# google-research/big_vision

Measured on NVIDIA H100. Metric: siglip_vit_b16_pairs_per_sec, higher is better.
Workload: dtype bf16

## Files before the change

big_vision_b200/csrc/gemm.cu:

```cuda
#include "common.cuh"
#include "gemm_sched.h"
#include "host_utils.h"

#include <atomic>

#include <stdlib.h>
#include <string.h>

namespace bv {

namespace {

constexpr int BM = 128;
constexpr int BK = 64;
constexpr int A_STAGE_BYTES = BM * BK * 2;
constexpr int NUM_THREADS = 384;
constexpr int SUB_BYTES = 64 * 64 * 2;

enum : int { EF_BIAS = 0, EF_GELU = 1, EF_RESID = 2, EF_DGELU = 3, EF_RESID_ROWMOD = 4, EF_GELU_ACT = 5 };
enum : int { OM_F32 = 0, OM_BF16_ADD = 1, OM_BF16_TMA = 2 };

template <int BN, int OM, int EF>
struct Cfg {
  static constexpr int B_STAGE_BYTES = BN * BK * 2;
  static constexpr int STAGE_BYTES = A_STAGE_BYTES + B_STAGE_BYTES;
  static constexpr bool AUX_TMA = OM == OM_BF16_TMA && (EF == EF_RESID || EF == EF_DGELU);
  static constexpr int OUTS = OM != OM_BF16_TMA ? 0 : (EF == EF_GELU ? 2 : 1);
  static constexpr int BUF_BYTES = OUTS * SUB_BYTES;
  static constexpr int BUFS = AUX_TMA ? BN / 64 : 2;
  static constexpr int STAGING_BYTES = 2 * BUFS * BUF_BYTES;
  static constexpr int SMEM_LIMIT = 232448 - 2048;
  static constexpr int STAGES_FIT = (SMEM_LIMIT - STAGING_BYTES) / STAGE_BYTES;
  static constexpr int STAGES = STAGES_FIT > 8 ? 8 : STAGES_FIT;
  static constexpr int STAGING_OFFSET = STAGES * STAGE_BYTES;
  static constexpr int BAR_OFFSET = STAGING_OFFSET + STAGING_BYTES;
  static constexpr int AUX_BAR = 2 * STAGES;
  static constexpr int SMEM_BYTES = BAR_OFFSET + 256 + 1024;
  static_assert(STAGES >= 3, "shared-memory budget leaves fewer than 3 stages");
  static_assert(8 * (AUX_BAR + (AUX_TMA ? 2 * BUFS : 0)) <= 256, "barriers overflow their 256 bytes");
};

struct GemmDev {
  GemmSched s;
  int M, N;
  int a_mn, b_mn;
  int reduce_out;
  float alpha;
  const float* bias;
  const bf16* aux;
  void* d; void* d2;
  long long ldd, ldd2, ldaux;
  float* colsum;
  int aux_row_mod;
};

template <int BN, int STAGES, int STAGE_BYTES, int TA, int TB, typename F>
__device__ __forceinline__ void mainloop(float (&acc)[BN / 2], uint32_t base, uint32_t bar_base, int cw,
                                         PipeState& ps, int kb0, int kb1, F&& after_first) {
  constexpr uint32_t a_lbo = TA ? 8192u : 16u, b_lbo = TB ? 8192u : 16u;
  constexpr uint32_t a_kstep = TA ? 2048u : 32u, b_kstep = TB ? 2048u : 32u;
  int prev_stage = -1;
  for (int kb = kb0; kb < kb1; ++kb) {
    mbar_wait(bar_base + 8u * ps.stage, ps.phase);
    const uint32_t a_s = base + ps.stage * STAGE_BYTES + cw * 8192;
    const uint32_t b_s = base + ps.stage * STAGE_BYTES + A_STAGE_BYTES;
    const uint64_t adesc = wgmma_desc_sw128(a_s, a_lbo, 1024u), bdesc = wgmma_desc_sw128(b_s, b_lbo, 1024u);
    wgmma_fence_regs(acc);
    wgmma_fence();
#pragma unroll
    for (int k = 0; k < BK / 16; ++k) {
      const uint64_t a = adesc + k * (a_kstep >> 4), b = bdesc + k * (b_kstep >> 4);
      const int accumulate = (kb > kb0 || k > 0) ? 1 : 0;
      if constexpr (BN == 256) wgmma_ss_n256<TA, TB>(acc, a, b, accumulate);
      else wgmma_ss_n128<TA, TB>(acc, a, b, accumulate);
    }
    wgmma_commit();
    wgmma_fence_regs(acc);
    if (kb == kb0) after_first();
    wgmma_wait<1>();
    if (prev_stage >= 0 && (threadIdx.x & 127) == 0) mbar_arrive(bar_base + 8u * (STAGES + prev_stage));
    prev_stage = ps.stage;
    ps.advance(STAGES);
  }
  wgmma_wait<0>();
  wgmma_fence_regs(acc);
  if (prev_stage >= 0 && (threadIdx.x & 127) == 0) mbar_arrive(bar_base + 8u * (STAGES + prev_stage));
}

__device__ __forceinline__ void aux_global(const GemmDev& p, int row, int col, bool pair, float& a0, float& a1) {
  const long long ar = p.aux_row_mod > 0 ? (row % p.aux_row_mod) : row;
  const bf16* ap = p.aux + ar * p.ldaux + col;
  if (pair) {
    const uint32_t q = *reinterpret_cast<const uint32_t*>(ap);
    a0 = bf16_lo(q); a1 = bf16_hi(q);
  } else {
    a0 = __bfloat162float(*ap);
    a1 = 0.f;
  }
}

template <bool OUT_F32, int EF>
__device__ __forceinline__ void epi_math(float alpha, float c0, float c1, float b0, float b1, float a0, float a1,
                                         float& v0, float& v1, float& pre0, float& pre1) {
  v0 = c0 * alpha + b0;
  v1 = c1 * alpha + b1;
  pre0 = pre1 = 0.f;
  if (EF == EF_GELU || EF == EF_GELU_ACT) {
    pre0 = round_bf16(v0); pre1 = round_bf16(v1);
    v0 = gelu_tanh_fast(pre0); v1 = gelu_tanh_fast(pre1);
  } else if (EF == EF_RESID || EF == EF_RESID_ROWMOD) {
    v0 = (OUT_F32 ? v0 : round_bf16(v0)) + a0;
    v1 = (OUT_F32 ? v1 : round_bf16(v1)) + a1;
  } else if (EF == EF_DGELU) {
    v0 *= gelu_tanh_grad_fast(a0);
    v1 *= gelu_tanh_grad_fast(a1);
  }
}


__device__ __forceinline__ void colsum_add(float* colsum, int N, float s0, float s1, int col, int lane) {
  s0 += __shfl_xor_sync(0xffffffffu, s0, 4);
  s0 += __shfl_xor_sync(0xffffffffu, s0, 8);
  s0 += __shfl_xor_sync(0xffffffffu, s0, 16);
  s1 += __shfl_xor_sync(0xffffffffu, s1, 4);
  s1 += __shfl_xor_sync(0xffffffffu, s1, 8);
  s1 += __shfl_xor_sync(0xffffffffu, s1, 16);
  if (lane < 4) {
    if (col < N) atomicAdd(colsum + col, s0);
    if (col + 1 < N) atomicAdd(colsum + col + 1, s1);
  }
}

template <int BN, bool OUT_F32, int EF>
__device__ __forceinline__ void epilogue_regs(const GemmDev& p, const float (&acc)[BN / 2], int m0, int n0,
                                              int cw, int kb0) {
  const int lane = threadIdx.x & 31, warp = (threadIdx.x >> 5) & 3;
  const int row0 = m0 + cw * 64 + warp * 16 + (lane >> 2);
  const int pM = p.M, pN = p.N;
  const float alpha = p.alpha;
  const bool reduce = p.reduce_out != 0;
  const bool first = kb0 == 0;
#pragma unroll
  for (int j = 0; j < BN / 8; ++j) {
    const int col = n0 + 8 * j + 2 * (lane & 3);
    if (col >= pN) continue;
    const bool pair = col + 1 < pN;
    float b0 = 0.f, b1 = 0.f;
    if (p.bias != nullptr && first) {
      b0 = __ldg(p.bias + col);
      if (pair) b1 = __ldg(p.bias + col + 1);
    }
#pragma unroll
    for (int h = 0; h < 2; ++h) {
      const int row = row0 + 8 * h;
      if (row >= pM) continue;
      float v0, v1, pre0, pre1, a0 = 0.f, a1 = 0.f;
      if ((EF == EF_RESID && first) || EF == EF_DGELU) aux_global(p, row, col, pair, a0, a1);
      epi_math<OUT_F32, EF>(alpha, acc[4 * j + 2 * h], acc[4 * j + 2 * h + 1], b0, b1, a0, a1, v0, v1, pre0, pre1);
      if (OUT_F32) {
        float* dp = static_cast<float*>(p.d) + row * p.ldd + col;
        if (reduce) {
          atomicAdd(dp, v0);
          if (pair) atomicAdd(dp + 1, v1);
        } else if (pair) {
          *reinterpret_cast<float2*>(dp) = make_float2(v0, v1);
        } else {
          *dp = v0;
        }
      } else {
        bf16* dp = static_cast<bf16*>(p.d) + row * p.ldd + col;
        const __nv_bfloat162 o = __floats2bfloat162_rn(v0, v1);
        if (pair) atomicAdd(reinterpret_cast<__nv_bfloat162*>(dp), o);
        else atomicAdd(dp, o.x);
      }
    }
  }
}

template <int BN, int EF, int BUF_BYTES>
__device__ __forceinline__ void epilogue_tma(const GemmDev& p, const CUtensorMap* tmD, const CUtensorMap* tmD2,
                                             const float (&acc)[BN / 2], int m0, int n0, int cw, uint32_t staging,
                                             uint32_t& nstore, uint32_t aux_bar, uint32_t aux_parity) {
  constexpr bool AUX_TMA = (EF == EF_RESID || EF == EF_DGELU);
  const int lane = threadIdx.x & 31, warp = (threadIdx.x >> 5) & 3;
  const bool leader = (threadIdx.x & 127) == 0;
  const int rl0 = warp * 16 + (lane >> 2);
  const int row0 = m0 + cw * 64 + rl0;
  const int pM = p.M, pN = p.N, pN8 = p.N & ~7;
  const float alpha = p.alpha;
#pragma unroll
  for (int c = 0; c < BN / 64; ++c) {
    uint32_t buf;
    if constexpr (AUX_TMA) {
      buf = staging + c * BUF_BYTES;
      mbar_wait(aux_bar + 8u * c, aux_parity);
    } else {
      buf = staging + (nstore & 1u) * BUF_BYTES;
      if (leader) tma_store_wait_read<1>();
      named_bar_sync(1 + cw, 128);
    }
    float cs[8][2];
#pragma unroll
    for (int jj = 0; jj < 8; ++jj) {
      const int j = 8 * c + jj;
      const int col = n0 + 8 * j + 2 * (lane & 3);
      cs[jj][0] = cs[jj][1] = 0.f;
      const bool cin = col < pN, pair = col + 1 < pN;
      float b0 = 0.f, b1 = 0.f;
      if (cin && p.bias != nullptr) {
        b0 = __ldg(p.bias + col);
        if (pair) b1 = __ldg(p.bias + col + 1);
      }
#pragma unroll
      for (int h = 0; h < 2; ++h) {
        const int rl = rl0 + 8 * h, row = row0 + 8 * h;
        const uint32_t off = rl * 128 + ((jj ^ (rl & 7)) << 4) + (lane & 3) * 4;
        float v0 = 0.f, v1 = 0.f, pre0 = 0.f, pre1 = 0.f;
        const bool in = cin && row < pM;
        if (in) {
          float a0 = 0.f, a1 = 0.f;
          if constexpr (AUX_TMA) {
            uint32_t q;
            asm volatile("ld.shared.b32 %0, [%1];" : "=r"(q) : "r"(buf + off));
            a0 = bf16_lo(q); a1 = bf16_hi(q);
          } else if constexpr (EF == EF_RESID_ROWMOD) {
            aux_global(p, row, col, pair, a0, a1);
          }
          epi_math<false, EF>(alpha, acc[4 * j + 2 * h], acc[4 * j + 2 * h + 1], b0, b1, a0, a1, v0, v1, pre0, pre1);
        }
        const __nv_bfloat162 o = __floats2bfloat162_rn(v0, v1);
        if (in) {
          cs[jj][0] += __low2float(o);
          cs[jj][1] += pair ? __high2float(o) : 0.f;
        }
        asm volatile("st.shared.b32 [%0], %1;" ::"r"(buf + off), "r"(*reinterpret_cast<const uint32_t*>(&o))
                     : "memory");
        if (EF == EF_GELU) {
          const __nv_bfloat162 q = __floats2bfloat162_rn(pre0, pre1);
          asm volatile("st.shared.b32 [%0], %1;" ::"r"(buf + SUB_BYTES + off),
                       "r"(*reinterpret_cast<const uint32_t*>(&q))
                       : "memory");
        }
      }
    }
    fence_proxy_async();
    named_bar_sync(1 + cw, 128);
    if (leader) {
      if (n0 + 64 * c < pN8 && m0 + cw * 64 < pM) {
        tma_store_2d(tmD, buf, n0 + 64 * c, m0 + cw * 64);
        if (EF == EF_GELU) tma_store_2d(tmD2, buf + SUB_BYTES, n0 + 64 * c, m0 + cw * 64);
      }
      tma_store_commit();
    }
    const int tail0 = pN8 - (n0 + 64 * c);
    if (pN8 < pN && tail0 >= 0 && tail0 < 64) {
      const int t = threadIdx.x & 127, rl = t & 63, out = t >> 6;
      const int row = m0 + cw * 64 + rl;
      if (row < pM && (out == 0 || EF == EF_GELU)) {
        const uint32_t src = buf + out * SUB_BYTES + rl * 128 + (((tail0 >> 3) ^ (rl & 7)) << 4);
        uint16_t* dst = reinterpret_cast<uint16_t*>(out ? p.d2 : p.d) + row * (out ? p.ldd2 : p.ldd) + pN8;
#pragma unroll 1
        for (int e = 0; e < pN - pN8; ++e) {
          uint16_t u;
          asm volatile("ld.shared.u16 %0, [%1];" : "=h"(u) : "r"(src + 2 * e));
          dst[e] = u;
        }
      }
      named_bar_sync(1 + cw, 128);
    }
    if (!AUX_TMA) ++nstore;
    if (p.colsum != nullptr) {
#pragma unroll
      for (int jj = 0; jj < 8; ++jj)
        colsum_add(p.colsum, pN, cs[jj][0], cs[jj][1], n0 + 8 * (8 * c + jj) + 2 * (lane & 3), lane);
    }
  }
}

template <int BN>
__device__ __forceinline__ void issue_aux_loads(const CUtensorMap* tmAux, int M, int N, int m0, int n0, int cw,
                                                uint32_t staging, uint32_t aux_bar) {
  tma_store_wait_read<0>();
#pragma unroll
  for (int c = 0; c < BN / 64; ++c) {
    const uint32_t bar = aux_bar + 8u * c;
    if (n0 + 64 * c < N && m0 + cw * 64 < M) {
      mbar_expect_tx(bar, SUB_BYTES);
      tma_load_2d(staging + c * SUB_BYTES, tmAux, bar, n0 + 64 * c, m0 + cw * 64);
    } else {
      mbar_arrive(bar);
    }
  }
}

template <int BN, int OM, int EF>
__global__ void __launch_bounds__(NUM_THREADS, 1)
gemm_kernel(const __grid_constant__ CUtensorMap tmA, const __grid_constant__ CUtensorMap tmB,
            const __grid_constant__ CUtensorMap tmD, const __grid_constant__ CUtensorMap tmD2,
            const __grid_constant__ CUtensorMap tmAux, const GemmDev p) {
  using C = Cfg<BN, OM, EF>;
  extern __shared__ uint8_t smem_raw[];
  const uint32_t raw_addr = smem_u32(smem_raw);
  const uint32_t base = (raw_addr + 1023u) & ~1023u;
  const uint32_t bar_base = base + C::BAR_OFFSET;
  auto full_bar = [&](int s) { return bar_base + 8u * s; };
  auto empty_bar = [&](int s) { return bar_base + 8u * (C::STAGES + s); };

  const int wg = __shfl_sync(0xffffffffu, static_cast<int>(threadIdx.x >> 7), 0);
  const int units = p.s.units;

  if (threadIdx.x == 0) {
    tma_prefetch_desc(&tmA);
    tma_prefetch_desc(&tmB);
    if (C::AUX_TMA) tma_prefetch_desc(&tmAux);
    for (int s = 0; s < C::STAGES; ++s) {
      mbar_init(full_bar(s), 1);
      mbar_init(empty_bar(s), 2);
    }
    if (C::AUX_TMA) {
      for (int b = 0; b < 2 * C::BUFS; ++b) mbar_init(bar_base + 8u * (C::AUX_BAR + b), 1);
    }
    fence_barrier_init();
  }
  __syncthreads();

  if (wg == 0) {
    asm volatile("setmaxnreg.dec.sync.aligned.u32 40;");
    if (threadIdx.x == 0) {
      PipeState ps;
      for (int u = blockIdx.x; u < units; u += gridDim.x) {
        const WorkUnit w = gemm_work_unit(p.s, u, BM, BN);
        for (int kb = w.kb0; kb < w.kb1; ++kb) {
          mbar_wait(empty_bar(ps.stage), ps.phase ^ 1u);
          const uint32_t a_s = base + ps.stage * C::STAGE_BYTES;
          const uint32_t b_s = a_s + A_STAGE_BYTES;
          const uint32_t fb = full_bar(ps.stage);
          mbar_expect_tx(fb, C::STAGE_BYTES);
          const int k0 = kb * BK;
          if (p.a_mn) {
#pragma unroll
            for (int j = 0; j < BM / 64; ++j) tma_load_2d(a_s + j * 8192, &tmA, fb, w.m0 + 64 * j, k0);
          } else {
            tma_load_2d(a_s, &tmA, fb, k0, w.m0);
          }
          if (p.b_mn) {
#pragma unroll
            for (int j = 0; j < BN / 64; ++j) tma_load_2d(b_s + j * 8192, &tmB, fb, w.n0 + 64 * j, k0);
          } else {
            tma_load_2d(b_s, &tmB, fb, k0, w.n0);
          }
          ps.advance(C::STAGES);
        }
      }
    }
    return;
  }

  asm volatile("setmaxnreg.inc.sync.aligned.u32 232;");
  const int cw = wg - 1;
  const uint32_t staging = base + C::STAGING_OFFSET + cw * C::BUFS * C::BUF_BYTES;
  const uint32_t aux_bar = bar_base + 8u * (C::AUX_BAR + cw * C::BUFS);
  const bool leader = (threadIdx.x & 127) == 0;
  uint32_t nstore = 0, nunit = 0;
  PipeState ps;
  constexpr int S = C::STAGES, SB = C::STAGE_BYTES;
  for (int u = blockIdx.x; u < units; u += gridDim.x, ++nunit) {
    const WorkUnit w = gemm_work_unit(p.s, u, BM, BN);
    auto after_first = [&]() {
      if constexpr (C::AUX_TMA) {
        if (leader) issue_aux_loads<BN>(&tmAux, p.M, p.N, w.m0, w.n0, cw, staging, aux_bar);
      }
    };
    float acc[BN / 2];
    if (p.a_mn) {
      if (p.b_mn) mainloop<BN, S, SB, 1, 1>(acc, base, bar_base, cw, ps, w.kb0, w.kb1, after_first);
      else mainloop<BN, S, SB, 1, 0>(acc, base, bar_base, cw, ps, w.kb0, w.kb1, after_first);
    } else {
      if (p.b_mn) mainloop<BN, S, SB, 0, 1>(acc, base, bar_base, cw, ps, w.kb0, w.kb1, after_first);
      else mainloop<BN, S, SB, 0, 0>(acc, base, bar_base, cw, ps, w.kb0, w.kb1, after_first);
    }

    if constexpr (OM == OM_BF16_TMA)
      epilogue_tma<BN, EF, C::BUF_BYTES>(p, &tmD, &tmD2, acc, w.m0, w.n0, cw, staging, nstore, aux_bar, nunit & 1u);
    else epilogue_regs<BN, OM == OM_F32, EF>(p, acc, w.m0, w.n0, cw, w.kb0);
  }
  if (OM == OM_BF16_TMA && (threadIdx.x & 127) == 0) tma_store_wait<0>();
}

template <int BN, int OM, int EF>
int launch_cfg(const bv_gemm_args& g, cudaStream_t stream) {
  using C = Cfg<BN, OM, EF>;
  CUtensorMap tmA, tmB, tmD, tmD2, tmAux;
  int rc;
  const CUtensorMapDataType bf = CU_TENSOR_MAP_DATA_TYPE_BFLOAT16;
  if (g.a_mn) rc = make_tmap_2d(&tmA, bf, g.A, g.M, g.K, g.lda * 2, 64, 64);
  else        rc = make_tmap_2d(&tmA, bf, g.A, g.K, g.M, g.lda * 2, 64, BM);
  if (rc) return rc;
  if (g.b_mn) rc = make_tmap_2d(&tmB, bf, g.B, g.N, g.K, g.ldb * 2, 64, 64);
  else        rc = make_tmap_2d(&tmB, bf, g.B, g.K, g.N, g.ldb * 2, 64, BN);
  if (rc) return rc;

  GemmDev p;
  const long long tiles = ((g.M + BM - 1) / BM) * ((g.N + BN - 1) / BN);
  if (tiles * ((g.K + BK - 1) / BK) > 0x7fffffffLL) { set_error("bv_gemm: problem too large"); return BV_ERR_INVALID; }
  if (!gemm_make_sched(g.M, g.N, g.K, BM, BN, BK, g.splits, g.reduce_out != 0, num_sms(), &p.s)) {
    set_error("bv_gemm: split-K requires reduce_out=1");
    return BV_ERR_INVALID;
  }
  p.M = (int)g.M; p.N = (int)g.N;
  p.a_mn = g.a_mn; p.b_mn = g.b_mn; p.reduce_out = g.reduce_out;
  p.alpha = g.alpha;
  p.bias = g.epilogue == BV_EPI_NONE ? nullptr : g.bias;
  p.colsum = g.colsum;
  p.aux = reinterpret_cast<const bf16*>(g.aux);
  p.ldaux = g.ldaux;
  p.aux_row_mod = g.aux_row_mod;
  p.d = g.D; p.d2 = g.D2;
  p.ldd = g.ldd; p.ldd2 = g.ldd2;
  memset(&tmD, 0, sizeof(tmD));
  memset(&tmD2, 0, sizeof(tmD2));
  memset(&tmAux, 0, sizeof(tmAux));
  const long long n8 = g.N & ~7LL;
  if (OM == OM_BF16_TMA && n8 > 0) {
    rc = make_tmap_2d(&tmD, bf, g.D, n8, g.M, g.ldd * 2, 64, 64);
    if (rc) return rc;
    if (EF == EF_GELU) {
      rc = make_tmap_2d(&tmD2, bf, g.D2, n8, g.M, g.ldd2 * 2, 64, 64);
      if (rc) return rc;
    }
  }
  if (C::AUX_TMA) {
    rc = make_tmap_2d(&tmAux, bf, g.aux, g.N, g.M, g.ldaux * 2, 64, 64);
    if (rc) return rc;
  }

  auto kern = gemm_kernel<BN, OM, EF>;
  static std::atomic<bool> attr_set[64];
  int dev = 0;
  if (cudaGetDevice(&dev) != cudaSuccess || dev < 0 || dev >= 64) dev = -1;
  if (dev < 0 || !attr_set[dev].load(std::memory_order_acquire)) {
    rc = check_cuda(cudaFuncSetAttribute(kern, cudaFuncAttributeMaxDynamicSharedMemorySize, C::SMEM_BYTES),
                    "cudaFuncSetAttribute(gemm)");
    if (rc) return rc;
    if (dev >= 0) attr_set[dev].store(true, std::memory_order_release);
  }
  const int grid = p.s.units < num_sms() ? p.s.units : num_sms();
  kern<<<grid, NUM_THREADS, C::SMEM_BYTES, stream>>>(tmA, tmB, tmD, tmD2, tmAux, p);
  return check_cuda(cudaGetLastError(), "gemm_kernel launch");
}

template <int BN>
int dispatch_epi(const bv_gemm_args& g, cudaStream_t s) {
  const bool f32 = (g.out_dtype == DT_F32), add = !f32 && g.reduce_out;
  switch (g.epilogue) {
    case BV_EPI_NONE:
    case BV_EPI_BIAS:
      return f32 ? launch_cfg<BN, OM_F32, EF_BIAS>(g, s)
                 : add ? launch_cfg<128, OM_BF16_ADD, EF_BIAS>(g, s) : launch_cfg<BN, OM_BF16_TMA, EF_BIAS>(g, s);
    case BV_EPI_BIAS_RESID:
      if (f32) return launch_cfg<BN, OM_F32, EF_RESID>(g, s);
      if (add) return launch_cfg<128, OM_BF16_ADD, EF_RESID>(g, s);
      return g.aux_row_mod > 0 ? launch_cfg<BN, OM_BF16_TMA, EF_RESID_ROWMOD>(g, s)
                               : launch_cfg<BN, OM_BF16_TMA, EF_RESID>(g, s);
    case BV_EPI_BIAS_GELU:
      return launch_cfg<BN, OM_BF16_TMA, EF_GELU>(g, s);
    case BV_EPI_BIAS_GELU_ACT:
      return launch_cfg<BN, OM_BF16_TMA, EF_GELU_ACT>(g, s);
    case BV_EPI_DGELU:
      if (f32) { set_error("bv_gemm: DGELU epilogue writes bf16"); return BV_ERR_INVALID; }
      if (g.aux_row_mod > 0) { set_error("bv_gemm: DGELU takes a row-aligned aux"); return BV_ERR_INVALID; }
      return add ? launch_cfg<128, OM_BF16_ADD, EF_DGELU>(g, s) : launch_cfg<BN, OM_BF16_TMA, EF_DGELU>(g, s);
  }
  set_error("bv_gemm: bad epilogue %d", g.epilogue);
  return BV_ERR_INVALID;
}

}
}

extern "C" {

int bv_gemm(const bv_gemm_args* args, void* stream) {
  using namespace bv;
  const cudaStream_t s = static_cast<cudaStream_t>(stream);
  if (!args) { set_error("bv_gemm: null args"); return BV_ERR_INVALID; }
  const bv_gemm_args& g = *args;
  if (g.M <= 0 || g.N <= 0 || g.K <= 0) { set_error("bv_gemm: empty problem"); return BV_ERR_INVALID; }
  if (g.out_dtype == DT_BF16 && ((reinterpret_cast<uintptr_t>(g.D) & 15) || (g.ldd % 8))) {
    set_error("bv_gemm: bf16 output must be 16B aligned with ldd %% 8 == 0"); return BV_ERR_INVALID;
  }
  if (g.out_dtype == DT_F32 && ((reinterpret_cast<uintptr_t>(g.D) & 7) || (g.ldd % 2))) {
    set_error("bv_gemm: fp32 output must be 8B aligned with an even ldd"); return BV_ERR_INVALID;
  }
  if (g.M > 0x7fffffffLL || g.N > 0x7fffffffLL || g.K > 0x7fffffffLL) {
    set_error("bv_gemm: dimension exceeds int32"); return BV_ERR_INVALID;
  }
  if (g.epilogue < BV_EPI_NONE || g.epilogue > BV_EPI_BIAS_GELU_ACT) {
    set_error("bv_gemm: bad epilogue %d", g.epilogue); return BV_ERR_INVALID;
  }
  if ((g.epilogue == BV_EPI_BIAS_RESID || g.epilogue == BV_EPI_DGELU) && g.aux == nullptr) {
    set_error("bv_gemm: epilogue %d needs aux", g.epilogue); return BV_ERR_INVALID;
  }
  if (g.aux != nullptr && ((reinterpret_cast<uintptr_t>(g.aux) & 15) || (g.ldaux % 8))) {
    set_error("bv_gemm: aux must be 16B aligned with ldaux %% 8 == 0"); return BV_ERR_INVALID;
  }
  if (g.bias != nullptr && (reinterpret_cast<uintptr_t>(g.bias) & 15)) {
    set_error("bv_gemm: bias must be 16B aligned"); return BV_ERR_INVALID;
  }
  if (g.epilogue == BV_EPI_BIAS_GELU && (g.out_dtype != DT_BF16 || g.D2 == nullptr || g.reduce_out)) {
    set_error("bv_gemm: BIAS_GELU needs bf16 output, D2 and no reduce"); return BV_ERR_INVALID;
  }
  if (g.epilogue == BV_EPI_BIAS_GELU && ((reinterpret_cast<uintptr_t>(g.D2) & 15) || (g.ldd2 % 8))) {
    set_error("bv_gemm: D2 must be 16B aligned with ldd2 %% 8 == 0"); return BV_ERR_INVALID;
  }
  if (g.epilogue == BV_EPI_BIAS_GELU_ACT && (g.out_dtype != DT_BF16 || g.reduce_out)) {
    set_error("bv_gemm: BIAS_GELU_ACT needs bf16 output and no reduce"); return BV_ERR_INVALID;
  }
  if (g.out_dtype != DT_F32 && g.out_dtype != DT_BF16) { set_error("bv_gemm: bad out dtype"); return BV_ERR_INVALID; }
  if (g.colsum != nullptr && (g.out_dtype != DT_BF16 || g.reduce_out)) {
    set_error("bv_gemm: colsum needs a plain bf16 output"); return BV_ERR_INVALID;
  }
  int bn = g.block_n;
  if (bn == 0) bn = (g.N > 128) ? 256 : 128;
  if (bn == 256) return dispatch_epi<256>(g, s);
  if (bn == 128) return dispatch_epi<128>(g, s);
  set_error("bv_gemm: block_n must be 0, 128 or 256");
  return BV_ERR_INVALID;
}

}
```

big_vision_b200/csrc/gemm_sched.h:

```cpp
#pragma once

#ifdef __CUDACC__
#define BV_HD __host__ __device__ __forceinline__
#else
#define BV_HD inline
#endif

namespace bv {

struct GemmSched {
  int num_m, num_n;
  int kblocks_total;
  int kblocks_per_split;
  int splits;
  int units;
};

struct WorkUnit {
  int m0, n0;
  int kb0, kb1;
};

inline bool gemm_make_sched(long long M, long long N, long long K, int bm, int bn, int bk, int splits_req,
                            bool reduce_out, int slots, GemmSched* s) {
  s->num_m = static_cast<int>((M + bm - 1) / bm);
  s->num_n = static_cast<int>((N + bn - 1) / bn);
  s->kblocks_total = static_cast<int>((K + bk - 1) / bk);
  int splits = splits_req;
  if (splits <= 0) {
    splits = 1;
    if (reduce_out) {
      const int tiles = s->num_m * s->num_n;
      int smax = s->kblocks_total / 16;
      if (smax > 32) smax = 32;
      double best = -1.0;
      for (int sp = 1; sp <= smax; ++sp) {
        const int units = tiles * sp;
        const int waves = (units + slots - 1) / slots;
        const double eff = static_cast<double>(units) / (static_cast<double>(waves) * slots) - 0.002 * sp;
        if (eff > best + 1e-9) { best = eff; splits = sp; }
      }
    }
  }
  if (splits > s->kblocks_total) splits = s->kblocks_total;
  if (splits < 1) splits = 1;
  if (splits > 1 && !reduce_out) return false;
  s->kblocks_per_split = (s->kblocks_total + splits - 1) / splits;
  s->splits = (s->kblocks_total + s->kblocks_per_split - 1) / s->kblocks_per_split;
  s->units = s->num_m * s->num_n * s->splits;
  return true;
}

BV_HD WorkUnit gemm_work_unit(const GemmSched& s, int u, int bm, int bn) {
  const int tiles = s.num_m * s.num_n;
  const int split = u / tiles, t = u - split * tiles;
  const int mt = t / s.num_n, nt = t - mt * s.num_n;
  WorkUnit w;
  w.m0 = mt * bm;
  w.n0 = nt * bn;
  w.kb0 = split * s.kblocks_per_split;
  w.kb1 = w.kb0 + s.kblocks_per_split < s.kblocks_total ? w.kb0 + s.kblocks_per_split : s.kblocks_total;
  return w;
}

struct PipeState {
  int stage = 0;
  unsigned phase = 0;
  BV_HD void advance(int stages) {
    if (++stage == stages) { stage = 0; phase ^= 1u; }
  }
};

}
```

Measured before the change: 2789.

## Add ping-pong consumer warpgroup scheduling for BN=128 GEMM tiles

For BN=128 tiles, each consumer warpgroup now computes a whole 128x128 tile (two 64-row halves) and the two warpgroups alternate work units. Issue barriers order their mainloops so one warpgroup's epilogue overlaps the other's MMA. bf16 outputs now default to BN=128 so they take this path, and the bf16 atomic epilogue uses an inline red.global.add instruction. This doubles the accumulator registers per warpgroup and adds cross-warpgroup barrier ordering, which could reduce occupancy or serialize mainloops.

```diff
diff --git a/big_vision_b200/csrc/gemm.cu b/big_vision_b200/csrc/gemm.cu
--- a/big_vision_b200/csrc/gemm.cu
+++ b/big_vision_b200/csrc/gemm.cu
@@ -22,12 +22,14 @@
 
 template <int BN, int OM, int EF>
 struct Cfg {
+  static constexpr bool PINGPONG = BN == 128;
+  static constexpr int HALVES = PINGPONG ? 2 : 1;
   static constexpr int B_STAGE_BYTES = BN * BK * 2;
   static constexpr int STAGE_BYTES = A_STAGE_BYTES + B_STAGE_BYTES;
   static constexpr bool AUX_TMA = OM == OM_BF16_TMA && (EF == EF_RESID || EF == EF_DGELU);
   static constexpr int OUTS = OM != OM_BF16_TMA ? 0 : (EF == EF_GELU ? 2 : 1);
   static constexpr int BUF_BYTES = OUTS * SUB_BYTES;
-  static constexpr int BUFS = AUX_TMA ? BN / 64 : 2;
+  static constexpr int BUFS = AUX_TMA ? HALVES * BN / 64 : 2;
   static constexpr int STAGING_BYTES = 2 * BUFS * BUF_BYTES;
   static constexpr int SMEM_LIMIT = 232448 - 2048;
   static constexpr int STAGES_FIT = (SMEM_LIMIT - STAGING_BYTES) / STAGE_BYTES;
@@ -35,9 +37,10 @@
   static constexpr int STAGING_OFFSET = STAGES * STAGE_BYTES;
   static constexpr int BAR_OFFSET = STAGING_OFFSET + STAGING_BYTES;
   static constexpr int AUX_BAR = 2 * STAGES;
+  static constexpr int ISSUED_BAR = AUX_BAR + (AUX_TMA ? 2 * BUFS : 0);
   static constexpr int SMEM_BYTES = BAR_OFFSET + 256 + 1024;
   static_assert(STAGES >= 3, "shared-memory budget leaves fewer than 3 stages");
-  static_assert(8 * (AUX_BAR + (AUX_TMA ? 2 * BUFS : 0)) <= 256, "barriers overflow their 256 bytes");
+  static_assert(8 * (ISSUED_BAR + 2) <= 256, "barriers overflow their 256 bytes");
 };
 
 struct GemmDev {
@@ -54,36 +57,48 @@
   int aux_row_mod;
 };
 
-template <int BN, int STAGES, int STAGE_BYTES, int TA, int TB, typename F>
-__device__ __forceinline__ void mainloop(float (&acc)[BN / 2], uint32_t base, uint32_t bar_base, int cw,
-                                         PipeState& ps, int kb0, int kb1, F&& after_first) {
+template <int BN, int H, int STAGES, int STAGE_BYTES, int TA, int TB, typename F, typename G>
+__device__ __forceinline__ void mainloop(float (&acc)[H][BN / 2], uint32_t base, uint32_t bar_base, int h0,
+                                         PipeState& ps, int kb0, int kb1, F&& after_first, G&& after_last) {
   constexpr uint32_t a_lbo = TA ? 8192u : 16u, b_lbo = TB ? 8192u : 16u;
   constexpr uint32_t a_kstep = TA ? 2048u : 32u, b_kstep = TB ? 2048u : 32u;
   int prev_stage = -1;
   for (int kb = kb0; kb < kb1; ++kb) {
     mbar_wait(bar_base + 8u * ps.stage, ps.phase);
-    const uint32_t a_s = base + ps.stage * STAGE_BYTES + cw * 8192;
+    const uint32_t a_s = base + ps.stage * STAGE_BYTES + h0 * 8192;
     const uint32_t b_s = base + ps.stage * STAGE_BYTES + A_STAGE_BYTES;
-    const uint64_t adesc = wgmma_desc_sw128(a_s, a_lbo, 1024u), bdesc = wgmma_desc_sw128(b_s, b_lbo, 1024u);
-    wgmma_fence_regs(acc);
+    const uint64_t bdesc = wgmma_desc_sw128(b_s, b_lbo, 1024u);
+    uint64_t adesc[H];
+#pragma unroll
+    for (int h = 0; h < H; ++h) {
+      adesc[h] = wgmma_desc_sw128(a_s + h * 8192, a_lbo, 1024u);
+      wgmma_fence_regs(acc[h]);
+    }
     wgmma_fence();
 #pragma unroll
     for (int k = 0; k < BK / 16; ++k) {
-      const uint64_t a = adesc + k * (a_kstep >> 4), b = bdesc + k * (b_kstep >> 4);
+      const uint64_t b = bdesc + k * (b_kstep >> 4);
       const int accumulate = (kb > kb0 || k > 0) ? 1 : 0;
-      if constexpr (BN == 256) wgmma_ss_n256<TA, TB>(acc, a, b, accumulate);
-      else wgmma_ss_n128<TA, TB>(acc, a, b, accumulate);
+#pragma unroll
+      for (int h = 0; h < H; ++h) {
+        const uint64_t a = adesc[h] + k * (a_kstep >> 4);
+        if constexpr (BN == 256) wgmma_ss_n256<TA, TB>(acc[h], a, b, accumulate);
+        else wgmma_ss_n128<TA, TB>(acc[h], a, b, accumulate);
+      }
     }
     wgmma_commit();
-    wgmma_fence_regs(acc);
+#pragma unroll
+    for (int h = 0; h < H; ++h) wgmma_fence_regs(acc[h]);
     if (kb == kb0) after_first();
+    if (kb == kb1 - 1) after_last();
     wgmma_wait<1>();
     if (prev_stage >= 0 && (threadIdx.x & 127) == 0) mbar_arrive(bar_base + 8u * (STAGES + prev_stage));
     prev_stage = ps.stage;
     ps.advance(STAGES);
   }
   wgmma_wait<0>();
-  wgmma_fence_regs(acc);
+#pragma unroll
+  for (int h = 0; h < H; ++h) wgmma_fence_regs(acc[h]);
   if (prev_stage >= 0 && (threadIdx.x & 127) == 0) mbar_arrive(bar_base + 8u * (STAGES + prev_stage));
 }
 
@@ -132,10 +147,10 @@
 }
 
 template <int BN, bool OUT_F32, int EF>
-__device__ __forceinline__ void epilogue_regs(const GemmDev& p, const float (&acc)[BN / 2], int m0, int n0,
-                                              int cw, int kb0) {
+__device__ __forceinline__ void epilogue_regs(const GemmDev& p, const float (&acc)[BN / 2], int r0, int n0,
+                                              int kb0) {
   const int lane = threadIdx.x & 31, warp = (threadIdx.x >> 5) & 3;
-  const int row0 = m0 + cw * 64 + warp * 16 + (lane >> 2);
+  const int row0 = r0 + warp * 16 + (lane >> 2);
   const int pM = p.M, pN = p.N;
   const float alpha = p.alpha;
   const bool reduce = p.reduce_out != 0;
@@ -169,9 +184,17 @@
         }
       } else {
         bf16* dp = static_cast<bf16*>(p.d) + row * p.ldd + col;
-        const __nv_bfloat162 o = __floats2bfloat162_rn(v0, v1);
-        if (pair) atomicAdd(reinterpret_cast<__nv_bfloat162*>(dp), o);
-        else atomicAdd(dp, o.x);
+        const uint32_t o = pack_bf16(v0, v1);
+        asm volatile(
+            "{\n"
+            ".reg .pred p;\n"
+            ".reg .b16 lo, hi;\n"
+            "setp.ne.u32 p, %2, 0;\n"
+            "mov.b32 {lo, hi}, %1;\n"
+            "@p red.global.add.noftz.bf16x2 [%0], %1;\n"
+            "@!p red.global.add.noftz.bf16 [%0], lo;\n"
+            "}\n" ::"l"(dp), "r"(o), "r"(pair ? 1u : 0u)
+            : "memory");
       }
     }
   }
@@ -179,13 +202,13 @@
 
 template <int BN, int EF, int BUF_BYTES>
 __device__ __forceinline__ void epilogue_tma(const GemmDev& p, const CUtensorMap* tmD, const CUtensorMap* tmD2,
-                                             const float (&acc)[BN / 2], int m0, int n0, int cw, uint32_t staging,
+                                             const float (&acc)[BN / 2], int r0, int n0, int cw, uint32_t staging,
                                              uint32_t& nstore, uint32_t aux_bar, uint32_t aux_parity) {
   constexpr bool AUX_TMA = (EF == EF_RESID || EF == EF_DGELU);
   const int lane = threadIdx.x & 31, warp = (threadIdx.x >> 5) & 3;
   const bool leader = (threadIdx.x & 127) == 0;
   const int rl0 = warp * 16 + (lane >> 2);
-  const int row0 = m0 + cw * 64 + rl0;
+  const int row0 = r0 + rl0;
   const int pM = p.M, pN = p.N, pN8 = p.N & ~7;
   const float alpha = p.alpha;
 #pragma unroll
@@ -246,16 +269,16 @@
     fence_proxy_async();
     named_bar_sync(1 + cw, 128);
     if (leader) {
-      if (n0 + 64 * c < pN8 && m0 + cw * 64 < pM) {
-        tma_store_2d(tmD, buf, n0 + 64 * c, m0 + cw * 64);
-        if (EF == EF_GELU) tma_store_2d(tmD2, buf + SUB_BYTES, n0 + 64 * c, m0 + cw * 64);
+      if (n0 + 64 * c < pN8 && r0 < pM) {
+        tma_store_2d(tmD, buf, n0 + 64 * c, r0);
+        if (EF == EF_GELU) tma_store_2d(tmD2, buf + SUB_BYTES, n0 + 64 * c, r0);
       }
       tma_store_commit();
     }
     const int tail0 = pN8 - (n0 + 64 * c);
     if (pN8 < pN && tail0 >= 0 && tail0 < 64) {
       const int t = threadIdx.x & 127, rl = t & 63, out = t >> 6;
-      const int row = m0 + cw * 64 + rl;
+      const int row = r0 + rl;
       if (row < pM && (out == 0 || EF == EF_GELU)) {
         const uint32_t src = buf + out * SUB_BYTES + rl * 128 + (((tail0 >> 3) ^ (rl & 7)) << 4);
         uint16_t* dst = reinterpret_cast<uint16_t*>(out ? p.d2 : p.d) + row * (out ? p.ldd2 : p.ldd) + pN8;
@@ -277,18 +300,23 @@
   }
 }
 
-template <int BN>
-__device__ __forceinline__ void issue_aux_loads(const CUtensorMap* tmAux, int M, int N, int m0, int n0, int cw,
+template <int BN, int H>
+__device__ __forceinline__ void issue_aux_loads(const CUtensorMap* tmAux, int M, int N, int m0, int n0, int h0,
                                                 uint32_t staging, uint32_t aux_bar) {
   tma_store_wait_read<0>();
 #pragma unroll
-  for (int c = 0; c < BN / 64; ++c) {
-    const uint32_t bar = aux_bar + 8u * c;
-    if (n0 + 64 * c < N && m0 + cw * 64 < M) {
-      mbar_expect_tx(bar, SUB_BYTES);
-      tma_load_2d(staging + c * SUB_BYTES, tmAux, bar, n0 + 64 * c, m0 + cw * 64);
-    } else {
-      mbar_arrive(bar);
+  for (int h = 0; h < H; ++h) {
+    const int r0 = m0 + 64 * (h0 + h);
+#pragma unroll
+    for (int c = 0; c < BN / 64; ++c) {
+      const int b = h * (BN / 64) + c;
+      const uint32_t bar = aux_bar + 8u * b;
+      if (n0 + 64 * c < N && r0 < M) {
+        mbar_expect_tx(bar, SUB_BYTES);
+        tma_load_2d(staging + b * SUB_BYTES, tmAux, bar, n0 + 64 * c, r0);
+      } else {
+        mbar_arrive(bar);
+      }
     }
   }
 }
@@ -315,10 +343,13 @@
     if (C::AUX_TMA) tma_prefetch_desc(&tmAux);
     for (int s = 0; s < C::STAGES; ++s) {
       mbar_init(full_bar(s), 1);
-      mbar_init(empty_bar(s), 2);
+      mbar_init(empty_bar(s), C::PINGPONG ? 1 : 2);
     }
     if (C::AUX_TMA) {
       for (int b = 0; b < 2 * C::BUFS; ++b) mbar_init(bar_base + 8u * (C::AUX_BAR + b), 1);
+    }
+    if (C::PINGPONG) {
+      for (int b = 0; b < 2; ++b) mbar_init(bar_base + 8u * (C::ISSUED_BAR + b), 1);
     }
     fence_barrier_init();
   }
@@ -358,33 +389,53 @@
 
   asm volatile("setmaxnreg.inc.sync.aligned.u32 232;");
   const int cw = wg - 1;
+  constexpr int H = C::HALVES;
+  const int h0 = C::PINGPONG ? 0 : cw;
   const uint32_t staging = base + C::STAGING_OFFSET + cw * C::BUFS * C::BUF_BYTES;
   const uint32_t aux_bar = bar_base + 8u * (C::AUX_BAR + cw * C::BUFS);
   const bool leader = (threadIdx.x & 127) == 0;
-  uint32_t nstore = 0, nunit = 0;
+  uint32_t nstore = 0;
   PipeState ps;
+  ConsumerWalk walk(blockIdx.x, gridDim.x, C::PINGPONG ? cw : -1);
+  WorkUnit w;
   constexpr int S = C::STAGES, SB = C::STAGE_BYTES;
-  for (int u = blockIdx.x; u < units; u += gridDim.x, ++nunit) {
-    const WorkUnit w = gemm_work_unit(p.s, u, BM, BN);
+  for (int j = 0; walk.next(p.s, BM, BN, S, ps, w); ++j) {
+    if constexpr (C::PINGPONG) {
+      const int prev = j + cw - 1;
+      if (prev >= 0) mbar_wait(bar_base + 8u * (C::ISSUED_BAR + 1 - cw), prev & 1);
+    }
     auto after_first = [&]() {
       if constexpr (C::AUX_TMA) {
-        if (leader) issue_aux_loads<BN>(&tmAux, p.M, p.N, w.m0, w.n0, cw, staging, aux_bar);
+        if (leader) issue_aux_loads<BN, H>(&tmAux, p.M, p.N, w.m0, w.n0, h0, staging, aux_bar);
       }
     };
-    float acc[BN / 2];
+    auto after_last = [&]() {
+      if constexpr (C::PINGPONG) {
+        if (leader) mbar_arrive(bar_base + 8u * (C::ISSUED_BAR + cw));
+      }
+    };
+    float acc[H][BN / 2];
     if (p.a_mn) {
-      if (p.b_mn) mainloop<BN, S, SB, 1, 1>(acc, base, bar_base, cw, ps, w.kb0, w.kb1, after_first);
-      else mainloop<BN, S, SB, 1, 0>(acc, base, bar_base, cw, ps, w.kb0, w.kb1, after_first);
+      if (p.b_mn) mainloop<BN, H, S, SB, 1, 1>(acc, base, bar_base, h0, ps, w.kb0, w.kb1, after_first, after_last);
+      else mainloop<BN, H, S, SB, 1, 0>(acc, base, bar_base, h0, ps, w.kb0, w.kb1, after_first, after_last);
     } else {
-      if (p.b_mn) mainloop<BN, S, SB, 0, 1>(acc, base, bar_base, cw, ps, w.kb0, w.kb1, after_first);
-      else mainloop<BN, S, SB, 0, 0>(acc, base, bar_base, cw, ps, w.kb0, w.kb1, after_first);
-    }
-
-    if constexpr (OM == OM_BF16_TMA)
-      epilogue_tma<BN, EF, C::BUF_BYTES>(p, &tmD, &tmD2, acc, w.m0, w.n0, cw, staging, nstore, aux_bar, nunit & 1u);
-    else epilogue_regs<BN, OM == OM_F32, EF>(p, acc, w.m0, w.n0, cw, w.kb0);
-  }
-  if (OM == OM_BF16_TMA && (threadIdx.x & 127) == 0) tma_store_wait<0>();
+      if (p.b_mn) mainloop<BN, H, S, SB, 0, 1>(acc, base, bar_base, h0, ps, w.kb0, w.kb1, after_first, after_last);
+      else mainloop<BN, H, S, SB, 0, 0>(acc, base, bar_base, h0, ps, w.kb0, w.kb1, after_first, after_last);
+    }
+
+#pragma unroll
+    for (int h = 0; h < H; ++h) {
+      const int r0 = w.m0 + 64 * (h0 + h);
+      if constexpr (OM == OM_BF16_TMA) {
+        const int b = C::AUX_TMA ? h * (BN / 64) : 0;
+        epilogue_tma<BN, EF, C::BUF_BYTES>(p, &tmD, &tmD2, acc[h], r0, w.n0, cw, staging + b * C::BUF_BYTES, nstore,
+                                           aux_bar + 8u * b, j & 1);
+      } else {
+        epilogue_regs<BN, OM == OM_F32, EF>(p, acc[h], r0, w.n0, w.kb0);
+      }
+    }
+  }
+  if (OM == OM_BF16_TMA && leader) tma_store_wait<0>();
 }
 
 template <int BN, int OM, int EF>
@@ -521,7 +572,7 @@
     set_error("bv_gemm: colsum needs a plain bf16 output"); return BV_ERR_INVALID;
   }
   int bn = g.block_n;
-  if (bn == 0) bn = (g.N > 128) ? 256 : 128;
+  if (bn == 0) bn = (g.N > 128 && g.out_dtype == DT_F32) ? 256 : 128;
   if (bn == 256) return dispatch_epi<256>(g, s);
   if (bn == 128) return dispatch_epi<128>(g, s);
   set_error("bv_gemm: block_n must be 0, 128 or 256");
diff --git a/big_vision_b200/csrc/gemm_sched.h b/big_vision_b200/csrc/gemm_sched.h
--- a/big_vision_b200/csrc/gemm_sched.h
+++ b/big_vision_b200/csrc/gemm_sched.h
@@ -69,6 +69,24 @@
   BV_HD void advance(int stages) {
     if (++stage == stages) { stage = 0; phase ^= 1u; }
   }
+  BV_HD void advance(int stages, int n) {
+    const int t = stage + n;
+    phase ^= static_cast<unsigned>(t / stages) & 1u;
+    stage = t % stages;
+  }
+};
+
+struct ConsumerWalk {
+  int unit, i, grid, cw;
+  BV_HD ConsumerWalk(int cta, int grid_, int cw_) : unit(cta - grid_), i(-1), grid(grid_), cw(cw_) {}
+  BV_HD bool next(const GemmSched& s, int bm, int bn, int stages, PipeState& ps, WorkUnit& w) {
+    for (unit += grid, ++i; unit < s.units; unit += grid, ++i) {
+      w = gemm_work_unit(s, unit, bm, bn);
+      if (cw < 0 || (i & 1) == cw) return true;
+      ps.advance(stages, w.kb1 - w.kb0);
+    }
+    return false;
+  }
 };
 
 }
```

New measurement: 2876 (median of 6 runs). 1.03x the previous value.
